# hhcho/sfgwas

Measured on AMD Instinct MI355X. Metric: pca_power_iter_ring_macs_per_s, higher is better.
Workload: dtype u64 ring words, exact integers: int8 digits on the matrix core for the MAC of all five moduli, fp64-held integers in the encode and key-switch kernels

## Files before the change

### sfgwas_amd/csrc/kernels.hpp

```cpp
#pragma once
#include "common.hpp"
#include "mm_plan.hpp"
#include "assoc_plan.hpp"

constexpr int SFG_MAXPATTERN = 128;
struct ModPattern { int period; int8_t m[SFG_MAXPATTERN]; };
struct RowMap { int rpg; size_t gstride_in, gstride_out; };
struct PanelMap { int G, g, shift0; unsigned packed_mask = 0; int K = 0; };

int launch_ntt_fwd(sfg_ctx *ctx, const u64 *in, u64 *out, size_t nrows, const ModPattern &pat);
int launch_ntt_inv(sfg_ctx *ctx, const u64 *in, u64 *out, size_t nrows, const ModPattern &pat);
int launch_ntt_plain(sfg_ctx *ctx, const double *pc, u64 *out, size_t nplain, int L);
struct MoveJob;
struct PtRide;
int launch_ntt_plain_half(sfg_ctx *ctx, const double *pc, u64 *out_half, size_t nplain, int L, PanelMap pm, const uint32_t *perm = nullptr, const MoveJob *mv = nullptr);
int launch_expand_half(sfg_ctx *ctx, const u64 *half, u64 *full, size_t nrows);
int launch_ntt_fwd_map(sfg_ctx *ctx, const u64 *in, u64 *out, size_t nrows, const ModPattern &pat, const RowMap &rm);
int launch_ntt_inv_map(sfg_ctx *ctx, const u64 *in, u64 *out, size_t nrows, const ModPattern &pat, const RowMap &rm);
int launch_ntt_fwd_staged(sfg_ctx *ctx, const u64 *in, u64 *out, size_t nrows, const ModPattern &pat, bool staged);
struct MacStrides { size_t rot_k, rot_r, pt_k, pt_n, out_n, out_r; bool pt_half = false; bool pt_packed = false; bool pt_digits = false; bool i8 = false; bool i8_big = false; bool pt_digits_big = false;
                    const int8_t *B_small = nullptr, *B_big = nullptr;
                    int pt_layout = 0, pt_L = 0;
                    int B_mode = 0;
                    const int8_t *A_small = nullptr, *A_big = nullptr; };
int launch_mac_i8_small(sfg_ctx *ctx, const double *rotf, size_t rotf_k_stride, size_t rotf_r_stride, int plane0, const u64 *pt, u64 *out, int K, int R, int r0, int Ncols,
                        int l0, int nl, int accumulate, const MacStrides &st);
int launch_mac_i8_big(sfg_ctx *ctx, const double *rotf, size_t rotf_k_stride, size_t rotf_r_stride, int plane0, const u64 *pt, u64 *out, int K, int R, int r0, int Ncols,
                      int l0, int accumulate, const MacStrides &st);
int launch_skew(sfg_ctx *ctx, const int8_t *blk, size_t ld, int r, int c, int transposed, int square, int8_t *D);
struct PcCache { double *slot = nullptr; int mode = 0; const uint32_t *perm = nullptr; };
int launch_encode_rows(sfg_ctx *ctx, const int8_t *D, int shift0, int nshift, int L, u64 *pt, bool half_rows = false, int G = 0, int g = 0, unsigned packed_mask = 0, const PcCache *pcache = nullptr,
                       PtRide *ride = nullptr);
int encode_rows_launches(const sfg_ctx *ctx, int nshift);
int i8_ride_prepare(sfg_ctx *ctx, const u64 *panel, int K, int Ncols, size_t pt_k, size_t pt_n, int layout, int L, int launches, PtRide &ride);
int i8_ride_finish(sfg_ctx *ctx, PtRide &ride);
int i8_ride_tiles(sfg_ctx *ctx, int K, int L, int8_t **Bs, int8_t **Bb);
struct I8Args;
void launch_i8_pack_pt_digits(hipStream_t q, const I8Args &a, unsigned items, bool big);
void launch_move_alone(hipStream_t q, const MoveJob &j);
int launch_share(sfg_ctx *ctx, const u64 *rows, size_t rows_ct_stride, const u64 *xr, size_t x_ct_stride, u64 *h, int nl, int nct);
int launch_add_rows(sfg_ctx *ctx, const u64 *a, size_t a_ct_stride, const u64 *b, size_t b_ct_stride, u64 *out, size_t out_ct_stride, int nl, int nct);
// ... 50 lines not shown
```

### sfgwas_amd/csrc/ntt.hip

```cpp
#include "common.hpp"
#include "kernels.hpp"
#include "i8_move.hpp"
#include "ntt_core.hpp"

template <int IN_MODE>
__global__ void __launch_bounds__(512) k_ntt_fwd(const void *in_, u64 *out_, ModPattern pat, RowMap rm, const double *tw_all, const double2 *pack_all, const ModConst *modc) {
    extern __shared__ double lds[];
    const int N = SFG_N, tid = threadIdx.x;
    const size_t row = blockIdx.x;
    const int m = pat.m[row % pat.period];
    const size_t grp = row / rm.rpg, gi = row % rm.rpg;
    if (m == -2) return;
    if (m < 0) {
        const u64 *src = (const u64 *)in_ + grp * rm.gstride_in + gi * N; u64 *dst = out_ + grp * rm.gstride_out + gi * N;
        if (IN_MODE == 0 && src != dst) for (int a = 0; a < 32; a++) dst[a * 512 + tid] = src[a * 512 + tid];
        return;
    }
    const double *tw = tw_all + (size_t)m * N;
    const double2 *pack = pack_all + (size_t)m * (N / 2);
    const double q = modc[m].q, qinv = modc[m].qinv;
    double v[32];
    if (IN_MODE == 0) {
        const u64 *in = (const u64 *)in_ + grp * rm.gstride_in + gi * N;
#pragma unroll
        for (int a = 0; a < 32; a++) v[a] = u64_to_f64(in[a * 512 + tid]);
    } else {
        const double *pc = (const double *)in_ + (row / pat.period) * (size_t)(N / 2);
#pragma unroll
        for (int a = 0; a < 16; a++) v[a] = pred(pc[a * 512 + tid], q, qinv);
#pragma unroll
        for (int a = 16; a < 32; a++) {
            int x = (a - 16) * 512 + tid;
            v[a] = x == 0 ? 0.0 : -pred(pc[N / 2 - x], q, qinv);
        }
    }
    ntt_fwd_phases(v, lds, tw, pack, q, qinv, tid);
    u64 *out = out_ + grp * rm.gstride_out + gi * N;
    {
        const int b = tid >> 4, c = tid & 15;
#pragma unroll
        for (int a = 0; a < 32; a++) out[a * 512 + tid] = f64_to_u64(canon(lds[a * LDS_ROW + c * 33 + b], q, qinv));
    }
}

__global__ void __launch_bounds__(512) k_ntt_inv(const u64 *in_, u64 *out_, ModPattern pat, RowMap rm, const double *tw_all, const double2 *pack_all, const ModConst *modc) {
    extern __shared__ double lds[];
    const int N = SFG_N, tid = threadIdx.x;
    const size_t row = blockIdx.x;
    const int m = pat.m[row % pat.period];
    if (m < 0) return;
    const size_t grp = row / rm.rpg, gi = row % rm.rpg;
    const double *tw = tw_all + (size_t)m * N;
    const double2 *pack = pack_all + (size_t)m * (N / 2);
    const double q = modc[m].q, qinv = modc[m].qinv;
    const u64 *in = in_ + grp * rm.gstride_in + gi * N;
    double v[32];
    {
        const int b = tid >> 4, c = tid & 15;
#pragma unroll
        for (int a = 0; a < 32; a++) lds[a * LDS_ROW + c * 33 + b] = u64_to_f64(in[a * 512 + tid]);
    }
    __syncthreads();
#pragma unroll
    for (int h = 0; h < 2; h++) {
        const int p = tid + 512 * h, a = p >> 5, b = p & 31;
        double w[16];
#pragma unroll
        for (int c = 0; c < 16; c++) w[c] = lds[a * LDS_ROW + c * 33 + b];
// ... 21 lines not shown
    {
        const int a = tid >> 4, c = tid & 15;
#pragma unroll
        for (int b = 0; b < 32; b++) v[b] = lds[a * LDS_ROW + c * 33 + b];
        gs_stage<32, 1>(v, q, qinv, [&](int g) { return tw[512 + a * 16 + g]; });
        gs_stage<32, 2>(v, q, qinv, [&](int g) { return tw[256 + a * 8 + g]; });
        gs_stage<32, 4>(v, q, qinv, [&](int g) { return tw[128 + a * 4 + g]; });
        gs_stage<32, 8>(v, q, qinv, [&](int g) { return tw[64 + a * 2 + g]; });
        gs_stage<32, 16>(v, q, qinv, [&](int g) { return tw[32 + a + g]; });
        __syncthreads();
#pragma unroll
        for (int b = 0; b < 32; b++) lds[a * LDS_ROW + b * 16 + c] = pred(v[b], q, qinv);
    }
    __syncthreads();
#pragma unroll
    for (int a = 0; a < 32; a++) v[a] = lds[a * LDS_ROW + tid];
    gs_stage<32, 1>(v, q, qinv, [&](int g) { return tw[16 + g]; });
    gs_stage<32, 2>(v, q, qinv, [&](int g) { return tw[8 + g]; });
    gs_stage<32, 4>(v, q, qinv, [&](int g) { return tw[4 + g]; });
    gs_stage<32, 8>(v, q, qinv, [&](int g) { return tw[2 + g]; });
    gs_stage<32, 16>(v, q, qinv, [&](int g) { return tw[1 + g]; });
    const double ninv = modc[m].ninv, ninv_q = modc[m].ninv_q;
    u64 *out = out_ + grp * rm.gstride_out + gi * N;
#pragma unroll
    for (int a = 0; a < 32; a++) {
        double x = mulmod_lazy(pred(v[a], q, qinv), ninv, ninv_q, q);
        out[a * 512 + tid] = f64_to_u64(canon(x, q, qinv));
    }
}

constexpr int H3_ROWA = 264;
constexpr int H3_WREG = 4 * 272;
constexpr int H3_DOUBLES = 16 * H3_ROWA > 4 * H3_WREG ? 16 * H3_ROWA : 4 * H3_WREG;
constexpr int H3_LDS_BYTES = H3_DOUBLES * 8;
struct NoFill {};
template <class First, class Store, class Fill = NoFill, bool WIDE = false>
__device__ __forceinline__ void ntt_half3_body(int hs, First first, Store store, double *lds, const double *tw, const double2 *pack, double q, double qinv, int tid, Fill fill = Fill()) {
    double v[32];
    const int a_b = tid >> 4, c_b = tid & 15;
    double w2[2][16];
    if constexpr (std::is_same<Fill, NoFill>::value) {
#pragma unroll
        for (int h = 0; h < 2; h++)
#pragma unroll
            for (int a = 0; a < 16; a++) w2[h][a] = first(a * 512 + tid + 256 * h);
    } else fill(w2);
// ... 201 lines not shown
    u64 *out = out_ + grp * rm.gstride_out + gi * N + (size_t)hs * n;
    if (m == -2) return;
    if (m < 0) {
        for (int k = 0; k < 32; k++) out[k * 256 + tid] = in[(size_t)hs * n + k * 256 + tid];
        return;
    }
    const double *tw = tw_all + (size_t)m * N;
    const double2 *pack = pack_all + (size_t)m * (N / 2);
    const double q = modc[m].q, qinv = modc[m].qinv;
    const double W = hs ? -tw[1] : tw[1], Wq = W * qinv;
    auto first = [&](int j) { return STAGED ? u64_to_f64(in[(size_t)hs * n + j]) : u64_to_f64(in[j]) + mulmod_lazy(u64_to_f64(in[n + j]), W, Wq, q); };
    ntt_half3_body(hs, first, [&](int j, double x) { out[j] = f64_to_u64(canon(x, q, qinv)); }, lds, tw, pack, q, qinv, tid);
}
__global__ void __launch_bounds__(256) k_expand_half(const u64 *half, u64 *full) {
    const int N = SFG_N, n = N / 2; const size_t row = blockIdx.x / (n / 256);
    const int i = (int)(blockIdx.x % (n / 256)) * 256 + threadIdx.x;
    const u64 v = half[row * n + i];
    full[row * N + i] = v; full[row * N + (N - 1 - i)] = v;
}

int ntt_set_attrs(sfg_ctx *ctx) {
    hipError_t e = hipFuncSetAttribute((const void *)k_ntt_fwd<0>, hipFuncAttributeMaxDynamicSharedMemorySize, LDS_DOUBLES * 8);
    if (e == hipSuccess) e = hipFuncSetAttribute((const void *)k_ntt_fwd<1>, hipFuncAttributeMaxDynamicSharedMemorySize, LDS_DOUBLES * 8);
    if (e == hipSuccess) e = hipFuncSetAttribute((const void *)k_ntt_inv, hipFuncAttributeMaxDynamicSharedMemorySize, LDS_DOUBLES * 8);
    if (e == hipSuccess) e = hipFuncSetAttribute((const void *)k_ntt_half3<false, false>, hipFuncAttributeMaxDynamicSharedMemorySize, H3_LDS_BYTES);
    if (e == hipSuccess) e = hipFuncSetAttribute((const void *)k_ntt_half3<true, false>, hipFuncAttributeMaxDynamicSharedMemorySize, H3_LDS_BYTES);
    if (e == hipSuccess) e = hipFuncSetAttribute((const void *)k_ntt_half3<false, true>, hipFuncAttributeMaxDynamicSharedMemorySize, H3_LDS_BYTES);
    if (e == hipSuccess) e = hipFuncSetAttribute((const void *)k_ntt_half3<true, true>, hipFuncAttributeMaxDynamicSharedMemorySize, H3_LDS_BYTES);
    if (e == hipSuccess) e = hipFuncSetAttribute((const void *)k_ntt_fwd_split<false>, hipFuncAttributeMaxDynamicSharedMemorySize, H3_LDS_BYTES);
    if (e == hipSuccess) e = hipFuncSetAttribute((const void *)k_ntt_fwd_split<true>, hipFuncAttributeMaxDynamicSharedMemorySize, H3_LDS_BYTES);
#define SFG_MV_ATTR(P, D, T) if (e == hipSuccess) e = hipFuncSetAttribute((const void *)k_ntt_half3_move<P, D, T>, hipFuncAttributeMaxDynamicSharedMemorySize, H3_LDS_BYTES)
    SFG_MV_ATTR(false, 1, true); SFG_MV_ATTR(true, 1, true);
#ifdef SFG_AB
    SFG_MV_ATTR(false, 1, false); SFG_MV_ATTR(false, 2, false); SFG_MV_ATTR(false, 2, true); SFG_MV_ATTR(false, 3, false); SFG_MV_ATTR(false, 3, true);
    SFG_MV_ATTR(true, 1, false); SFG_MV_ATTR(true, 2, false); SFG_MV_ATTR(true, 2, true); SFG_MV_ATTR(true, 3, false); SFG_MV_ATTR(true, 3, true);
    if (e == hipSuccess && ab_set_attrs(ctx)) return 1;
#endif
#undef SFG_MV_ATTR
    if (e != hipSuccess) SFG_FAIL(ctx, "cannot raise dynamic LDS limit for the NTT kernels");
    return 0;
}

static RowMap dense_map() { RowMap rm; rm.rpg = 1; rm.gstride_in = SFG_N; rm.gstride_out = SFG_N; return rm; }
int launch_ntt_fwd(sfg_ctx *ctx, const u64 *in, u64 *out, size_t nrows, const ModPattern &pat) { return launch_ntt_fwd_map(ctx, in, out, nrows, pat, dense_map()); }
int launch_ntt_inv(sfg_ctx *ctx, const u64 *in, u64 *out, size_t nrows, const ModPattern &pat) { return launch_ntt_inv_map(ctx, in, out, nrows, pat, dense_map()); }
int launch_ntt_fwd_map(sfg_ctx *ctx, const u64 *in, u64 *out, size_t nrows, const ModPattern &pat, const RowMap &rm) {
    if (!nrows) return 0;
// ... 41 lines not shown
        if (perm) SFG_TRY(launch_half3_move<true>(ctx, g2, pc, out_half, nplain, L, pm, perm, *mv));
        else SFG_TRY(launch_half3_move<false>(ctx, g2, pc, out_half, nplain, L, pm, (const uint32_t *)nullptr, *mv));
        SFG_HIP(ctx, hipGetLastError());
        return 0;
    }
    if (perm && dig) hipLaunchKernelGGL((k_ntt_half3<true, true>), grid, dim3(256), H3_LDS_BYTES, ctx->stream, pc, out_half, nplain, L, pm, ctx->tw_fwd, ctx->pack_fwd, ctx->modc, perm);
    else if (perm) hipLaunchKernelGGL((k_ntt_half3<true, false>), grid, dim3(256), H3_LDS_BYTES, ctx->stream, pc, out_half, nplain, L, pm, ctx->tw_fwd, ctx->pack_fwd, ctx->modc, perm);
    else if (dig) hipLaunchKernelGGL((k_ntt_half3<false, true>), grid, dim3(256), H3_LDS_BYTES, ctx->stream, pc, out_half, nplain, L, pm, ctx->tw_fwd, ctx->pack_fwd, ctx->modc, (const uint32_t *)nullptr);
#ifdef SFG_AB
    else if (ctx->cfg.ntt_half_full) ab_launch_ntt_half_full(ctx, pc, out_half, nplain, L, pm);
#endif
    else hipLaunchKernelGGL((k_ntt_half3<false, false>), grid, dim3(256), H3_LDS_BYTES, ctx->stream, pc, out_half, nplain, L, pm, ctx->tw_fwd, ctx->pack_fwd, ctx->modc, (const uint32_t *)nullptr);
    SFG_HIP(ctx, hipGetLastError());
    return 0;
}
int launch_expand_half(sfg_ctx *ctx, const u64 *half, u64 *full, size_t nrows) {
    if (!nrows) return 0;
    hipLaunchKernelGGL(k_expand_half, dim3((unsigned)(nrows * (SFG_N / 2 / 256))), dim3(256), 0, ctx->stream, half, full);
    SFG_HIP(ctx, hipGetLastError());
    return 0;
}
int launch_ntt_inv_map(sfg_ctx *ctx, const u64 *in, u64 *out, size_t nrows, const ModPattern &pat, const RowMap &rm) {
    if (!nrows) return 0;
    hipLaunchKernelGGL(k_ntt_inv, dim3((unsigned)nrows), dim3(512), LDS_DOUBLES * 8, ctx->stream, in, out, pat, rm, ctx->tw_inv, ctx->pack_inv, ctx->modc);
    SFG_HIP(ctx, hipGetLastError());
    return 0;
}

static int pattern_from_host(sfg_ctx *ctx, const int *mod_idx, int nrows, ModPattern &pat) {
    for (int period = 1; period <= 64 && period <= nrows; period++) {
        bool ok = true;
        for (int r = 0; r < nrows && ok; r++) ok = mod_idx[r] == mod_idx[r % period];
        if (ok) { pat.period = period; for (int i = 0; i < period; i++) { if (mod_idx[i] < 0 || mod_idx[i] >= ctx->nmod) SFG_FAIL(ctx, "modulus index out of range"); pat.m[i] = (int8_t)mod_idx[i]; } return 0; }
    }
    SFG_FAIL(ctx, "mod_idx must be periodic with period <= 64");
}

extern "C" int sfg_ntt_rows(sfg_ctx *ctx, uint64_t *rows, int nrows, const int *mod_idx) {
    SFG_HIP(ctx, hipSetDevice(ctx->device));
    ModPattern pat; SFG_TRY(pattern_from_host(ctx, mod_idx, nrows, pat));
    return launch_ntt_fwd(ctx, (const u64 *)rows, (u64 *)rows, nrows, pat);
}
extern "C" int sfg_intt_rows(sfg_ctx *ctx, uint64_t *rows, int nrows, const int *mod_idx) {
    SFG_HIP(ctx, hipSetDevice(ctx->device));
    ModPattern pat; SFG_TRY(pattern_from_host(ctx, mod_idx, nrows, pat));
    return launch_ntt_inv(ctx, (const u64 *)rows, (u64 *)rows, nrows, pat);
}
// ... 1 lines not shown
```

### sfgwas_amd/csrc/rotate.hip

```cpp
#include "common.hpp"
#include "kernels.hpp"
#include "ksw.hpp"


static void fill_ext(const sfg_ctx *ctx, ExtConst &e, const std::vector<int> &src) {
    memset(&e, 0, sizeof e);
    e.a = (int)src.size();
    for (int m = 0; m < e.a; m++) e.src[m] = src[m];
    for (int m = 0; m < e.a; m++) {
        u64 qm = ctx->q[src[m]], h = 1;
        for (int k = 0; k < e.a; k++) if (k != m) h = h_mulmod(h, ctx->q[src[k]] % qm, qm);
        u64 hi = h_invmod(h, qm);
        e.qhat_inv[m] = (double)hi; e.qhat_inv_q[m] = (double)hi / (double)qm;
    }
    for (int t = 0; t < ctx->nmod; t++) {
        u64 qt = ctx->q[t], D = 1 % qt;
        for (int m = 0; m < e.a; m++) {
            u64 ht = 1 % qt;
            for (int k = 0; k < e.a; k++) if (k != m) ht = h_mulmod(ht, ctx->q[src[k]] % qt, qt);
            e.qhat_t[t][m] = (double)ht; e.qhat_t_q[t][m] = (double)ht / (double)qt;
            D = h_mulmod(D, ctx->q[src[m]] % qt, qt);
        }
        e.D_t[t] = (double)D; e.D_t_q[t] = (double)D / (double)qt;
    }
}
// ... 111 lines not shown
    } else o[x] = (ff.centre && v > __builtin_floor(q * 0.5)) ? v - q : v;
}
__global__ void __launch_bounds__(256) k_ksw_finish(const u64 *ct_in, const int *inidx, const u64 *acc, const u64 *ext2, const uint16_t *const *index,
                                                   u64 *const *ct_out, const KswConst *kcp, const ModConst *modc, const u64 *add1, F64Form ff) {
    const KswConst &kc = *kcp;
    const int N = SFG_N, x = blockIdx.x * 256 + threadIdx.x, t = blockIdx.y; const size_t b = blockIdx.z;
    if (ff.on && t >= ff.L) return;
    const double q = modc[t].q, qinv = modc[t].qinv, pinv = kc.pinv[t], pinv_q = kc.pinv_q[t];
    const int src = index[b][x];
#pragma unroll
    for (int p = 0; p < 2; p++) {
        const double a = u64_to_f64(acc[((b * 2 + p) * (size_t)kc.nt + t) * N + src]);
        const double e = u64_to_f64(ext2[((b * 2 + p) * (size_t)kc.nl + t) * N + src]);
        double r = mulmod_lazy(a - e, pinv, pinv_q, q);
        if (p == 0) r += u64_to_f64(ct_in[((size_t)inidx[b] * 2 * (size_t)kc.nl + t) * N + src]);
        else if (add1) r += u64_to_f64(add1[((size_t)inidx[b] * (size_t)kc.nl + t) * N + src]);
        const double v = canon(r, q, qinv);
        if (ff.on) store_rot_f64(reinterpret_cast<double *>(ct_out[b]) + (size_t)p * ff.rowf, ff, t, x, v, q);
        else ct_out[b][((size_t)p * kc.nl + t) * N + x] = f64_to_u64(v);
    }
}

struct KswSeg { const u64 *plain; u64 *out; int start, count, accumulate, pad; };
__global__ void __launch_bounds__(256) k_ksw_finish_sum(const u64 *ct_in, const int *inidx, const u64 *acc, const u64 *ext2, const uint16_t *const *index,
                                                       const KswSeg *segs, const int *jobs, const KswConst *kcp, const ModConst *modc) {
    const KswConst &kc = *kcp;
    const int N = SFG_N, x = blockIdx.x * 256 + threadIdx.x, t = blockIdx.y;
    const KswSeg sg = segs[blockIdx.z];
    const double q = modc[t].q, qinv = modc[t].qinv, pinv = kc.pinv[t], pinv_q = kc.pinv_q[t];
    const size_t w0 = (size_t)t * N + x, w1 = ((size_t)kc.nl + t) * N + x;
    double s0 = 0.0, s1 = 0.0;
    if (sg.accumulate) { s0 = u64_to_f64(sg.out[w0]); s1 = u64_to_f64(sg.out[w1]); }
    if (sg.plain) { s0 += u64_to_f64(sg.plain[w0]); s1 += u64_to_f64(sg.plain[w1]); }
    for (int k = 0; k < sg.count; k++) {
        const size_t b = (size_t)jobs[sg.start + k];
        const int src = index[b][x];
        const double a0 = u64_to_f64(acc[((b * 2 + 0) * (size_t)kc.nt + t) * N + src]), e0 = u64_to_f64(ext2[((b * 2 + 0) * (size_t)kc.nl + t) * N + src]);
        const double a1 = u64_to_f64(acc[((b * 2 + 1) * (size_t)kc.nt + t) * N + src]), e1 = u64_to_f64(ext2[((b * 2 + 1) * (size_t)kc.nl + t) * N + src]);
        const double c0 = u64_to_f64(ct_in[((size_t)inidx[b] * 2 * (size_t)kc.nl + t) * N + src]);
        s0 += canon(mulmod_lazy(a0 - e0, pinv, pinv_q, q) + c0, q, qinv);
        s1 += canon(mulmod_lazy(a1 - e1, pinv, pinv_q, q), q, qinv);
        if ((k & 7) == 7) { s0 = pred(s0, q, qinv); s1 = pred(s1, q, qinv); }
    }
    sg.out[w0] = f64_to_u64(canon(s0, q, qinv)); sg.out[w1] = f64_to_u64(canon(s1, q, qinv));
}

__global__ void __launch_bounds__(256) k_ct_add(const u64 *a, const u64 *b, u64 *out, int nl, const ModConst *modc, size_t total_rows) {
    const int N = SFG_N; const size_t row = blockIdx.x / (N / 256); const int m = (int)(row % nl);
    const u64 q = modc[m].qi;
    const size_t off = row * N + (blockIdx.x % (N / 256)) * 256 + threadIdx.x;
    u64 v = a[off] + b[off]; out[off] = v >= q ? v - q : v;
}

struct KswSum { int nout; std::vector<int> group; std::vector<const u64 *> plain; u64 *out; size_t out_stride; int accumulate; };
static int launch_keyswitch_jobs(sfg_ctx *ctx, const u64 *in, int nin, int level, const std::vector<int> &job_in, const std::vector<const u64 *> &keyp,
                                 const std::vector<const uint16_t *> &idxp, const std::vector<u64 *> &outp, const u64 *add1, const F64Form *ffp = nullptr,
                                 const KswSum *sum = nullptr) {
    const int N = SFG_N, nl = level + 1;
    F64Form ff; memset(&ff, 0, sizeof ff); if (ffp) ff = *ffp;
    KswConst *kcd; KswConst kc;
    SFG_TRY(get_ksw(ctx, level, &kcd, &kc));
    const size_t ctw = (size_t)2 * nl * N;
    const int nr = (int)job_in.size(), nout = sum ? sum->nout : 0;
    if (sum && (ff.on || add1 || (int)sum->group.size() != nr || (int)sum->plain.size() != nout)) SFG_FAIL(ctx, "key switch: internal: malformed sum groups");
    if (!nr && !nout) return 0;
    const int nq_out = ff.on ? ff.L : nl;
    const bool pre1 = !ctx->cfg.ntt_fwd_full;
    const size_t in_rows = (size_t)nl + (size_t)kc.beta * kc.nt, job_rows = 2 * (size_t)kc.nt + 2 * (size_t)nl;
    const size_t budget = ctx->cfg.ksw_budget;
    int in_grp = (int)(budget / (in_rows * N * 8)); if (in_grp < 1) in_grp = 1; if (in_grp > nin) in_grp = nin;
    int chunk = (int)(budget / (job_rows * N * 8)); if (chunk < 1) chunk = 1; if (chunk > nr) chunk = nr;
    const size_t ptr_bytes = (size_t)nr * (3 * sizeof(void *) + 2 * sizeof(int)) + (size_t)nout * sizeof(KswSeg) + 256;
    const size_t ext_rows = (size_t)in_grp * kc.beta * kc.nt, ext2_rows = (size_t)chunk * 2 * nl;
    SFG_TRY(sfg_ws_reserve(ctx, (in_rows * in_grp + job_rows * chunk + ext_rows + ext2_rows) * N * 8 + ptr_bytes));
    u64 *c2 = (u64 *)ctx->ws, *ext = c2 + (size_t)in_grp * nl * N;
    u64 *acc = ext + ext_rows * N, *ext2 = acc + (size_t)chunk * 2 * kc.nt * N;
    u64 *extT = ext2 + ext2_rows * N, *ext2T = extT + ext_rows * N;
    const u64 **keys_all = (const u64 **)(ext2T + ext2_rows * N);
    const uint16_t **idx_all = (const uint16_t **)(keys_all + nr);
    u64 **out_all = (u64 **)(idx_all + nr);
    KswSeg *segs_d = (KswSeg *)(out_all + nr);
    int *inidx_all = (int *)(segs_d + nout);
    int *segjobs_d = inidx_all + nr;
    std::vector<char> seen(nout, 0);
    std::vector<KswSeg> segs; std::vector<int> segjobs;
    auto finish_sum = [&](const std::vector<int> &jobs, size_t c0, int nb, const u64 *bin, const int *inidx_d, const uint16_t **idx_d) -> int {
        std::vector<int> cnt(nout, 0), at(nout, 0);
        for (int k = 0; k < nb; k++) cnt[sum->group[jobs[c0 + k]]]++;
        segs.clear(); segjobs.assign(nb, 0);
        for (int i = 0, start = 0; i < nout; i++) {
            if (nb ? !cnt[i] : seen[i]) continue;
            KswSeg sg; sg.plain = seen[i] ? nullptr : sum->plain[i]; sg.out = sum->out + (size_t)i * sum->out_stride;
            sg.start = start; sg.count = cnt[i]; sg.accumulate = (sum->accumulate || seen[i]) ? 1 : 0; sg.pad = 0;
            at[i] = start; start += cnt[i]; seen[i] = 1; segs.push_back(sg);
        }
        for (int k = 0; k < nb; k++) segjobs[at[sum->group[jobs[c0 + k]]]++] = k;
        if (segs.empty()) return 0;
        SFG_TRY(sfg_upload_small(ctx, segs_d, segs.data(), segs.size() * sizeof(KswSeg)));
        SFG_TRY(sfg_upload_small(ctx, segjobs_d, segjobs.data(), (size_t)nb * sizeof(int)));
        hipLaunchKernelGGL(k_ksw_finish_sum, dim3(N / 256, nl, (unsigned)segs.size()), dim3(256), 0, ctx->stream, bin, inidx_d, acc, ext2T, idx_d, segs_d, segjobs_d, kcd, ctx->modc);
        SFG_HIP(ctx, hipGetLastError());
        return 0;
    };
    ModPattern pq; pq.period = nl; for (int m = 0; m < nl; m++) pq.m[m] = m < nq_out ? (int8_t)m : (int8_t)-2;
    ModPattern pin; pin.period = nl; for (int m = 0; m < nl; m++) pin.m[m] = (int8_t)m;
    ModPattern pext; pext.period = kc.beta * kc.nt;
    for (int i = 0; i < kc.beta; i++) for (int t = 0; t < kc.nt; t++)
        pext.m[i * kc.nt + t] = (kc.digit_of[t] == i || (t >= nq_out && t < nl)) ? (int8_t)-2 : (int8_t)kc.tmod[t];
    ModPattern pp; pp.period = kc.np; for (int p = 0; p < kc.np; p++) pp.m[p] = (int8_t)(ctx->nq + p);
    for (int i0 = 0; i0 < nin; i0 += in_grp) {
        const int ni = nin - i0 < in_grp ? nin - i0 : in_grp;
        std::vector<int> jobs;
        for (int k = 0; k < nr; k++) if (job_in[k] >= i0 && job_in[k] < i0 + ni) jobs.push_back(k);
        if (jobs.empty()) continue;
        const u64 *bin = in + (size_t)i0 * ctw;
        RowMap rm1; rm1.rpg = nl; rm1.gstride_in = ctw; rm1.gstride_out = (size_t)nl * N;
        SFG_TRY(launch_ntt_inv_map(ctx, bin + (size_t)nl * N, c2, (size_t)ni * nl, pin, rm1));
        if (pre1) hipLaunchKernelGGL(k_ksw_extend<true>, dim3(N / 512, kc.beta, ni), dim3(256), 0, ctx->stream, c2, ext, kcd, ctx->modc, ctx->tw_fwd);
        else hipLaunchKernelGGL(k_ksw_extend<false>, dim3(N / 512, kc.beta, ni), dim3(256), 0, ctx->stream, c2, ext, kcd, ctx->modc, ctx->tw_fwd);
        SFG_HIP(ctx, hipGetLastError());
        SFG_TRY(launch_ntt_fwd_staged(ctx, ext, extT, (size_t)ni * kc.beta * kc.nt, pext, pre1));
        {
            const size_t nj = jobs.size();
            std::vector<const u64 *> kp(nj); std::vector<const uint16_t *> ip(nj); std::vector<u64 *> op(nj); std::vector<int> ii(nj);
            for (size_t k = 0; k < nj; k++) { int jb = jobs[k]; kp[k] = keyp[jb]; ip[k] = idxp[jb]; op[k] = sum ? nullptr : outp[jb]; ii[k] = job_in[jb] - i0; }
            SFG_TRY(sfg_upload_small(ctx, keys_all, kp.data(), nj * sizeof(void *)));
            SFG_TRY(sfg_upload_small(ctx, idx_all, ip.data(), nj * sizeof(void *)));
            if (!sum) SFG_TRY(sfg_upload_small(ctx, out_all, op.data(), nj * sizeof(void *)));
            SFG_TRY(sfg_upload_small(ctx, inidx_all, ii.data(), nj * sizeof(int)));
        }
        for (size_t c0 = 0; c0 < jobs.size(); c0 += chunk) {
            const int nb = (int)(jobs.size() - c0 < (size_t)chunk ? jobs.size() - c0 : (size_t)chunk);
            const u64 **keys_d = keys_all + c0; const uint16_t **idx_d = idx_all + c0; u64 **out_d = out_all + c0; int *inidx_d = inidx_all + c0;
            hipLaunchKernelGGL(k_ksw_inner, dim3(N / 512, nq_out + kc.np, nb), dim3(256), 0, ctx->stream, extT, bin, keys_d, inidx_d, acc, kcd, ctx->modc, ctx->nmod, nq_out);
            SFG_HIP(ctx, hipGetLastError());
            RowMap rm4; rm4.rpg = kc.np; rm4.gstride_in = (size_t)kc.nt * N; rm4.gstride_out = (size_t)kc.nt * N;
            SFG_TRY(launch_ntt_inv_map(ctx, acc + (size_t)nl * N, acc + (size_t)nl * N, (size_t)nb * 2 * kc.np, pp, rm4));
            if (pre1) hipLaunchKernelGGL(k_moddown_extend<true>, dim3(N / 512, 2, nb), dim3(256), 0, ctx->stream, acc, ext2, kcd, ctx->modc, ctx->tw_fwd, nq_out);
            else hipLaunchKernelGGL(k_moddown_extend<false>, dim3(N / 512, 2, nb), dim3(256), 0, ctx->stream, acc, ext2, kcd, ctx->modc, ctx->tw_fwd, nq_out);
            SFG_HIP(ctx, hipGetLastError());
            SFG_TRY(launch_ntt_fwd_staged(ctx, ext2, ext2T, (size_t)nb * 2 * nl, pq, pre1));
            if (sum) { SFG_TRY(finish_sum(jobs, c0, nb, bin, inidx_d, idx_d)); continue; }
            hipLaunchKernelGGL(k_ksw_finish, dim3(N / 256, nq_out, nb), dim3(256), 0, ctx->stream, bin, inidx_d, acc, ext2T, idx_d, out_d, kcd, ctx->modc,
                               add1 ? add1 + (size_t)i0 * nl * N : nullptr, ff);
            SFG_HIP(ctx, hipGetLastError());
        }
    }
    if (sum) SFG_TRY(finish_sum(std::vector<int>(), 0, 0, in, inidx_all, idx_all));
    return 0;
}
int launch_rotate_right_indexed(sfg_ctx *ctx, const u64 *in, int nin, u64 *out, int nct, int level, const int *nrot_host, const int *in_index) {
    const int N = SFG_N, nl = level + 1;
    if (level < 0 || level >= ctx->nq) SFG_FAIL(ctx, "rotate: level out of range");
    const size_t ctw = (size_t)2 * nl * N;
    std::vector<int> job_in; std::vector<const u64 *> keyp; std::vector<const uint16_t *> idxp; std::vector<u64 *> outp;
    for (int j = 0; j < nct; j++) {
        int nrot = nrot_host[j] % SFG_SLOTS; if (nrot < 0) nrot += SFG_SLOTS;
        const int src = in_index ? in_index[j] : j;
        if (src < 0 || src >= nin) SFG_FAIL(ctx, "rotate: input index out of range");
        if (nrot == 0) {
            int run = 1;
            while (j + run < nct && (nrot_host[j + run] % SFG_SLOTS) == 0 && (in_index ? in_index[j + run] : j + run) == src + run && src + run < nin) run++;
            SFG_HIP(ctx, hipMemcpyAsync(out + j * ctw, in + (size_t)src * ctw, (size_t)run * ctw * 8, hipMemcpyDeviceToDevice, ctx->stream));
            j += run - 1;
            continue;
        }
        u64 g = sfg_galois_for_rotation(ctx, SFG_SLOTS - nrot);
        auto it = ctx->rotkeys().find(g);
        if (it == ctx->rotkeys().end()) SFG_FAIL(ctx, "rotate: no rotation key loaded for right-rotation by %d (galois element %llu)", nrot, g);
        job_in.push_back(src); keyp.push_back(it->second.key_dev); idxp.push_back(it->second.index_dev); outp.push_back(out + j * ctw);
    }
    return launch_keyswitch_jobs(ctx, in, nin, level, job_in, keyp, idxp, outp, nullptr);
}
int launch_rotate_right_sum(sfg_ctx *ctx, const u64 *in, int nin, int nct, int level, const int *nrot_host, const int *in_index, const int *group, int nout,
                            u64 *out, size_t out_stride, int accumulate) {
    const int N = SFG_N, nl = level + 1;
    if (level < 0 || level >= ctx->nq) SFG_FAIL(ctx, "rotate: level out of range");
    const size_t ctw = (size_t)2 * nl * N;
    KswSum sum; sum.nout = nout; sum.plain.assign(nout, nullptr); sum.out = out; sum.out_stride = out_stride; sum.accumulate = accumulate;
    std::vector<int> job_in; std::vector<const u64 *> keyp; std::vector<const uint16_t *> idxp;
    for (int j = 0; j < nct; j++) {
        int nrot = nrot_host[j] % SFG_SLOTS; if (nrot < 0) nrot += SFG_SLOTS;
        const int src = in_index ? in_index[j] : j;
        if (src < 0 || src >= nin) SFG_FAIL(ctx, "rotate: input index out of range");
        if (group[j] < 0 || group[j] >= nout) SFG_FAIL(ctx, "rotate: sum group out of range");
        if (nrot == 0) {
            if (sum.plain[group[j]]) SFG_FAIL(ctx, "rotate: more than one unrotated member in a sum group");
            sum.plain[group[j]] = in + (size_t)src * ctw;
            continue;
        }
        u64 g = sfg_galois_for_rotation(ctx, SFG_SLOTS - nrot);
        auto it = ctx->rotkeys().find(g);
        if (it == ctx->rotkeys().end()) SFG_FAIL(ctx, "rotate: no rotation key loaded for right-rotation by %d (galois element %llu)", nrot, g);
        job_in.push_back(src); keyp.push_back(it->second.key_dev); idxp.push_back(it->second.index_dev); sum.group.push_back(group[j]);
    }
    return launch_keyswitch_jobs(ctx, in, nin, level, job_in, keyp, idxp, std::vector<u64 *>(), nullptr, nullptr, &sum);
}
int launch_rotate_right_indexed_f64(sfg_ctx *ctx, const u64 *in, int nin, double *outf, int nct, int level, const int *nrot_host, const int *in_index, int L,
                                    const size_t *out_slot) {
    const int N = SFG_N, nl = level + 1;
    ctx->i8_gen++;
    if (level < 0 || level >= ctx->nq || L > nl) SFG_FAIL(ctx, "rotate: level out of range");
    const size_t ctw = (size_t)2 * nl * N;
    std::vector<int> plane_of, is_big; const int nplanes = mac_dma_planes(ctx, L, plane_of, is_big);
    if (nplanes < 0) return 1;
    F64Form ff; memset(&ff, 0, sizeof ff);
    ff.on = 1; ff.L = L; ff.centre = mac_dma_packed_mask(ctx, L) != 0; ff.rowf = (size_t)nplanes * N;
    for (int l = 0; l < L; l++) { ff.plane_of[l] = plane_of[l]; ff.big[l] = is_big[l]; }
    std::vector<int> job_in; std::vector<const u64 *> keyp; std::vector<const uint16_t *> idxp; std::vector<u64 *> outp;
    for (int j = 0; j < nct; j++) {
        int nrot = nrot_host[j] % SFG_SLOTS; if (nrot < 0) nrot += SFG_SLOTS;
        const int src = in_index ? in_index[j] : j;
        if (src < 0 || src >= nin) SFG_FAIL(ctx, "rotate: input index out of range");
        double *dst = outf + (out_slot ? out_slot[j] : (size_t)j) * 2 * ff.rowf;
        if (nrot == 0) {
            int run = 1;
            while (!out_slot && j + run < nct && (nrot_host[j + run] % SFG_SLOTS) == 0 && (in_index ? in_index[j + run] : j + run) == src + run && src + run < nin) run++;
// ... 61 lines not shown
```

Baseline: 6113 billion.

## Sum rotated key-switch outputs before mod-down by applying the Galois map in coefficient domain

For rotate-and-sum groups, the inverse NTT of the P-part now writes each coefficient at its Galois-permuted position and tags negated ones. A new kernel then does mod-down extension and summation across the group's jobs, split over a few partial sums, before a single forward NTT per partial. The finish kernel sums raw accumulators and divides by P once. This removes a forward NTT and an extension per job in exchange for a scatter through LDS, extra partial-sum buffers and more workspace.

Result: no change. 6156 billion (median of 6 runs) (+0.7%).

```diff
diff --git a/sfgwas_amd/csrc/galois_coeff.hpp b/sfgwas_amd/csrc/galois_coeff.hpp
--- /dev/null
+++ b/sfgwas_amd/csrc/galois_coeff.hpp
@@ -0,0 +1,12 @@
+#pragma once
+#include "fp64mod.hpp"
+
+SFG_HD void galois_coeff_dst(unsigned i, unsigned g, unsigned n, unsigned &j, unsigned &neg) {
+    const unsigned r = (i * g) & (2u * n - 1u);
+    j = r & (n - 1u); neg = r >= n ? 1u : 0u;
+}
+constexpr unsigned long long GALOIS_NEG = 1ull << 63;
+SFG_HD unsigned long long galois_tag(unsigned long long word, unsigned neg) { return neg ? word | GALOIS_NEG : word; }
+SFG_HD unsigned galois_neg_of(unsigned long long tagged) { return (unsigned)(tagged >> 63); }
+SFG_HD unsigned long long galois_word_of(unsigned long long tagged) { return tagged & ~GALOIS_NEG; }
+SFG_HD double galois_signed(double v, unsigned neg, double q) { return neg ? (v != 0.0 ? q - v : 0.0) : v; }
diff --git a/sfgwas_amd/csrc/kernels.hpp b/sfgwas_amd/csrc/kernels.hpp
--- a/sfgwas_amd/csrc/kernels.hpp
+++ b/sfgwas_amd/csrc/kernels.hpp
@@ -17,6 +17,7 @@
 int launch_expand_half(sfg_ctx *ctx, const u64 *half, u64 *full, size_t nrows);
 int launch_ntt_fwd_map(sfg_ctx *ctx, const u64 *in, u64 *out, size_t nrows, const ModPattern &pat, const RowMap &rm);
 int launch_ntt_inv_map(sfg_ctx *ctx, const u64 *in, u64 *out, size_t nrows, const ModPattern &pat, const RowMap &rm);
+int launch_ntt_inv_galois(sfg_ctx *ctx, const u64 *in, u64 *out, size_t nrows, const ModPattern &pat, const RowMap &rm, const unsigned *galois_dev, int gal_rows);
 int launch_ntt_fwd_staged(sfg_ctx *ctx, const u64 *in, u64 *out, size_t nrows, const ModPattern &pat, bool staged);
 struct MacStrides { size_t rot_k, rot_r, pt_k, pt_n, out_n, out_r; bool pt_half = false; bool pt_packed = false; bool pt_digits = false; bool i8 = false; bool i8_big = false; bool pt_digits_big = false;
                     const int8_t *B_small = nullptr, *B_big = nullptr;
diff --git a/sfgwas_amd/csrc/ntt.hip b/sfgwas_amd/csrc/ntt.hip
--- a/sfgwas_amd/csrc/ntt.hip
+++ b/sfgwas_amd/csrc/ntt.hip
@@ -2,6 +2,7 @@
 #include "kernels.hpp"
 #include "i8_move.hpp"
 #include "ntt_core.hpp"
+#include "galois_coeff.hpp"
 
 template <int IN_MODE>
 __global__ void __launch_bounds__(512) k_ntt_fwd(const void *in_, u64 *out_, ModPattern pat, RowMap rm, const double *tw_all, const double2 *pack_all, const ModConst *modc) {
@@ -43,7 +44,9 @@
     }
 }
 
-__global__ void __launch_bounds__(512) k_ntt_inv(const u64 *in_, u64 *out_, ModPattern pat, RowMap rm, const double *tw_all, const double2 *pack_all, const ModConst *modc) {
+template <bool GAL>
+__global__ void __launch_bounds__(512) k_ntt_inv(const u64 *in_, u64 *out_, ModPattern pat, RowMap rm, const double *tw_all, const double2 *pack_all, const ModConst *modc,
+                                                 const unsigned *galois, int gal_rows) {
     extern __shared__ double lds[];
     const int N = SFG_N, tid = threadIdx.x;
     const size_t row = blockIdx.x;
@@ -111,6 +114,21 @@
     gs_stage<32, 16>(v, q, qinv, [&](int g) { return tw[1 + g]; });
     const double ninv = modc[m].ninv, ninv_q = modc[m].ninv_q;
     u64 *out = out_ + grp * rm.gstride_out + gi * N;
+    if (GAL) {
+        const unsigned g = galois[row / (size_t)gal_rows];
+        u64 *img = reinterpret_cast<u64 *>(lds);
+        __syncthreads();
+#pragma unroll
+        for (int a = 0; a < 32; a++) {
+            double x = mulmod_lazy(pred(v[a], q, qinv), ninv, ninv_q, q);
+            unsigned j, neg; galois_coeff_dst((unsigned)(a * 512 + tid), g, (unsigned)N, j, neg);
+            img[(j >> 9) * LDS_ROW + (j & 511)] = galois_tag(f64_to_u64(canon(x, q, qinv)), neg);
+        }
+        __syncthreads();
+#pragma unroll
+        for (int a = 0; a < 32; a++) out[a * 512 + tid] = img[a * LDS_ROW + tid];
+        return;
+    }
 #pragma unroll
     for (int a = 0; a < 32; a++) {
         double x = mulmod_lazy(pred(v[a], q, qinv), ninv, ninv_q, q);
@@ -358,7 +376,8 @@
 int ntt_set_attrs(sfg_ctx *ctx) {
     hipError_t e = hipFuncSetAttribute((const void *)k_ntt_fwd<0>, hipFuncAttributeMaxDynamicSharedMemorySize, LDS_DOUBLES * 8);
     if (e == hipSuccess) e = hipFuncSetAttribute((const void *)k_ntt_fwd<1>, hipFuncAttributeMaxDynamicSharedMemorySize, LDS_DOUBLES * 8);
-    if (e == hipSuccess) e = hipFuncSetAttribute((const void *)k_ntt_inv, hipFuncAttributeMaxDynamicSharedMemorySize, LDS_DOUBLES * 8);
+    if (e == hipSuccess) e = hipFuncSetAttribute((const void *)k_ntt_inv<false>, hipFuncAttributeMaxDynamicSharedMemorySize, LDS_DOUBLES * 8);
+    if (e == hipSuccess) e = hipFuncSetAttribute((const void *)k_ntt_inv<true>, hipFuncAttributeMaxDynamicSharedMemorySize, LDS_DOUBLES * 8);
     if (e == hipSuccess) e = hipFuncSetAttribute((const void *)k_ntt_half3<false, false>, hipFuncAttributeMaxDynamicSharedMemorySize, H3_LDS_BYTES);
     if (e == hipSuccess) e = hipFuncSetAttribute((const void *)k_ntt_half3<true, false>, hipFuncAttributeMaxDynamicSharedMemorySize, H3_LDS_BYTES);
     if (e == hipSuccess) e = hipFuncSetAttribute((const void *)k_ntt_half3<false, true>, hipFuncAttributeMaxDynamicSharedMemorySize, H3_LDS_BYTES);
@@ -446,7 +465,14 @@
 }
 int launch_ntt_inv_map(sfg_ctx *ctx, const u64 *in, u64 *out, size_t nrows, const ModPattern &pat, const RowMap &rm) {
     if (!nrows) return 0;
-    hipLaunchKernelGGL(k_ntt_inv, dim3((unsigned)nrows), dim3(512), LDS_DOUBLES * 8, ctx->stream, in, out, pat, rm, ctx->tw_inv, ctx->pack_inv, ctx->modc);
+    hipLaunchKernelGGL(k_ntt_inv<false>, dim3((unsigned)nrows), dim3(512), LDS_DOUBLES * 8, ctx->stream, in, out, pat, rm, ctx->tw_inv, ctx->pack_inv, ctx->modc, (const unsigned *)nullptr, 1);
+    SFG_HIP(ctx, hipGetLastError());
+    return 0;
+}
+int launch_ntt_inv_galois(sfg_ctx *ctx, const u64 *in, u64 *out, size_t nrows, const ModPattern &pat, const RowMap &rm, const unsigned *galois_dev, int gal_rows) {
+    if (!nrows) return 0;
+    if (!galois_dev || gal_rows < 1) SFG_FAIL(ctx, "inverse NTT: the automorphism store needs a Galois element per job");
+    hipLaunchKernelGGL(k_ntt_inv<true>, dim3((unsigned)nrows), dim3(512), LDS_DOUBLES * 8, ctx->stream, in, out, pat, rm, ctx->tw_inv, ctx->pack_inv, ctx->modc, galois_dev, gal_rows);
     SFG_HIP(ctx, hipGetLastError());
     return 0;
 }
diff --git a/sfgwas_amd/csrc/rotate.hip b/sfgwas_amd/csrc/rotate.hip
--- a/sfgwas_amd/csrc/rotate.hip
+++ b/sfgwas_amd/csrc/rotate.hip
@@ -1,6 +1,7 @@
 #include "common.hpp"
 #include "kernels.hpp"
 #include "ksw.hpp"
+#include "galois_coeff.hpp"
 
 
 static void fill_ext(const sfg_ctx *ctx, ExtConst &e, const std::vector<int> &src) {
@@ -158,25 +159,81 @@
 }
 
 struct KswSeg { const u64 *plain; u64 *out; int start, count, accumulate, pad; };
-__global__ void __launch_bounds__(256) k_ksw_finish_sum(const u64 *ct_in, const int *inidx, const u64 *acc, const u64 *ext2, const uint16_t *const *index,
-                                                       const KswSeg *segs, const int *jobs, const KswConst *kcp, const ModConst *modc) {
+constexpr int KSW_SUM_PARTS = 8;
+constexpr int KSW_SUM_WGS = 4096;
+template <bool PRE1, int MAXT>
+__global__ void __launch_bounds__(256) k_moddown_extend_sum(const u64 *acc, u64 *esum, const KswSeg *segs, const int *jobs, const KswConst *kcp, const ModConst *modc,
+                                                           const double *tw_fwd, int nq_out, int nparts) {
+    const KswConst &kc = *kcp;
+    const int N = SFG_N, n = N / 2, x = blockIdx.x * 256 + threadIdx.x, p = blockIdx.y;
+    const KswSeg sg = segs[blockIdx.z / nparts];
+    const ExtConst &e = kc.pq;
+    double s[2][MAXT];
+#pragma unroll
+    for (int t = 0; t < MAXT; t++) s[0][t] = s[1][t] = 0.0;
+    for (int k = blockIdx.z % nparts, c = 0; k < sg.count; k += nparts, c++) {
+        const size_t b = (size_t)jobs[sg.start + k];
+        const u64 *ap = acc + ((b * 2 + p) * (size_t)kc.nt + kc.nl) * N;
+        double xs[2][KSW_MAXA], y[2][KSW_MAXA], v[2] = {0.0, 0.0};
+        unsigned neg[2] = {0u, 0u};
+#pragma unroll
+        for (int h = 0; h < 2; h++)
+#pragma unroll
+            for (int m = 0; m < KSW_MAXA; m++) {
+                const u64 w = m < e.a ? ap[(size_t)m * N + h * n + x] : 0;
+                xs[h][m] = u64_to_f64(galois_word_of(w));
+                if (m == 0) neg[h] = galois_neg_of(w);
+            }
+        if (e.a > 1) { ext_prepare(e, modc, xs[0], y[0], v[0]); ext_prepare(e, modc, xs[1], y[1], v[1]); }
+#pragma unroll
+        for (int t = 0; t < MAXT; t++) {
+            if (t < nq_out) {
+                const double q = modc[t].q, qinv = modc[t].qinv;
+                double o0, o1;
+                if (e.a == 1) { o0 = canon(xs[0][0], q, qinv); o1 = canon(xs[1][0], q, qinv); }
+                else { o0 = ext_target(e, t, q, qinv, y[0], v[0]); o1 = ext_target(e, t, q, qinv, y[1], v[1]); }
+                s[0][t] += galois_signed(o0, neg[0], q); s[1][t] += galois_signed(o1, neg[1], q);
+                if ((c & 7) == 7) { s[0][t] = pred(s[0][t], q, qinv); s[1][t] = pred(s[1][t], q, qinv); }
+            }
+        }
+    }
+#pragma unroll
+    for (int t = 0; t < MAXT; t++) {
+        if (t < nq_out) {
+            const double q = modc[t].q, qinv = modc[t].qinv;
+            double o0 = canon(s[0][t], q, qinv), o1 = canon(s[1][t], q, qinv);
+            if (PRE1) { const double W = tw_fwd[(size_t)t * N + 1]; fwd_stage1_pair(o0, o1, W, W * qinv, q, qinv, o0, o1); }
+            u64 *row = esum + (((size_t)blockIdx.z * 2 + p) * (size_t)kc.nl + t) * N;
+            row[x] = f64_to_u64(o0); row[n + x] = f64_to_u64(o1);
+        }
+    }
+}
+__global__ void __launch_bounds__(256) k_ksw_finish_sum(const u64 *ct_in, const int *inidx, const u64 *acc, const u64 *esumT, const uint16_t *const *index,
+                                                       const KswSeg *segs, const int *jobs, const KswConst *kcp, const ModConst *modc, int nparts) {
     const KswConst &kc = *kcp;
     const int N = SFG_N, x = blockIdx.x * 256 + threadIdx.x, t = blockIdx.y;
     const KswSeg sg = segs[blockIdx.z];
     const double q = modc[t].q, qinv = modc[t].qinv, pinv = kc.pinv[t], pinv_q = kc.pinv_q[t];
     const size_t w0 = (size_t)t * N + x, w1 = ((size_t)kc.nl + t) * N + x;
-    double s0 = 0.0, s1 = 0.0;
+    double s0 = 0.0, s1 = 0.0, a0 = 0.0, a1 = 0.0;
     if (sg.accumulate) { s0 = u64_to_f64(sg.out[w0]); s1 = u64_to_f64(sg.out[w1]); }
     if (sg.plain) { s0 += u64_to_f64(sg.plain[w0]); s1 += u64_to_f64(sg.plain[w1]); }
     for (int k = 0; k < sg.count; k++) {
         const size_t b = (size_t)jobs[sg.start + k];
         const int src = index[b][x];
-        const double a0 = u64_to_f64(acc[((b * 2 + 0) * (size_t)kc.nt + t) * N + src]), e0 = u64_to_f64(ext2[((b * 2 + 0) * (size_t)kc.nl + t) * N + src]);
-        const double a1 = u64_to_f64(acc[((b * 2 + 1) * (size_t)kc.nt + t) * N + src]), e1 = u64_to_f64(ext2[((b * 2 + 1) * (size_t)kc.nl + t) * N + src]);
-        const double c0 = u64_to_f64(ct_in[((size_t)inidx[b] * 2 * (size_t)kc.nl + t) * N + src]);
-        s0 += canon(mulmod_lazy(a0 - e0, pinv, pinv_q, q) + c0, q, qinv);
-        s1 += canon(mulmod_lazy(a1 - e1, pinv, pinv_q, q), q, qinv);
-        if ((k & 7) == 7) { s0 = pred(s0, q, qinv); s1 = pred(s1, q, qinv); }
+        a0 += u64_to_f64(acc[((b * 2 + 0) * (size_t)kc.nt + t) * N + src]);
+        a1 += u64_to_f64(acc[((b * 2 + 1) * (size_t)kc.nt + t) * N + src]);
+        s0 += u64_to_f64(ct_in[((size_t)inidx[b] * 2 * (size_t)kc.nl + t) * N + src]);
+        if ((k & 7) == 7) { a0 = pred(a0, q, qinv); a1 = pred(a1, q, qinv); s0 = pred(s0, q, qinv); }
+    }
+    if (sg.count) {
+        double e0 = 0.0, e1 = 0.0;
+        for (int r = 0; r < nparts; r++) {
+            e0 += u64_to_f64(esumT[((((size_t)blockIdx.z * nparts + r) * 2 + 0) * (size_t)kc.nl + t) * N + x]);
+            e1 += u64_to_f64(esumT[((((size_t)blockIdx.z * nparts + r) * 2 + 1) * (size_t)kc.nl + t) * N + x]);
+        }
+        s0 += mulmod_lazy(pred(a0, q, qinv) - e0, pinv, pinv_q, q);
+        s1 += mulmod_lazy(pred(a1, q, qinv) - e1, pinv, pinv_q, q);
     }
     sg.out[w0] = f64_to_u64(canon(s0, q, qinv)); sg.out[w1] = f64_to_u64(canon(s1, q, qinv));
 }
@@ -188,7 +245,7 @@
     u64 v = a[off] + b[off]; out[off] = v >= q ? v - q : v;
 }
 
-struct KswSum { int nout; std::vector<int> group; std::vector<const u64 *> plain; u64 *out; size_t out_stride; int accumulate; };
+struct KswSum { int nout; std::vector<int> group; std::vector<unsigned> galois; std::vector<const u64 *> plain; u64 *out; size_t out_stride; int accumulate; };
 static int launch_keyswitch_jobs(sfg_ctx *ctx, const u64 *in, int nin, int level, const std::vector<int> &job_in, const std::vector<const u64 *> &keyp,
                                  const std::vector<const uint16_t *> &idxp, const std::vector<u64 *> &outp, const u64 *add1, const F64Form *ffp = nullptr,
                                  const KswSum *sum = nullptr) {
@@ -198,7 +255,7 @@
     SFG_TRY(get_ksw(ctx, level, &kcd, &kc));
     const size_t ctw = (size_t)2 * nl * N;
     const int nr = (int)job_in.size(), nout = sum ? sum->nout : 0;
-    if (sum && (ff.on || add1 || (int)sum->group.size() != nr || (int)sum->plain.size() != nout)) SFG_FAIL(ctx, "key switch: internal: malformed sum groups");
+    if (sum && (ff.on || add1 || (int)sum->group.size() != nr || (int)sum->galois.size() != nr || (int)sum->plain.size() != nout)) SFG_FAIL(ctx, "key switch: internal: malformed sum groups");
     if (!nr && !nout) return 0;
     const int nq_out = ff.on ? ff.L : nl;
     const bool pre1 = !ctx->cfg.ntt_fwd_full;
@@ -206,9 +263,10 @@
     const size_t budget = ctx->cfg.ksw_budget;
     int in_grp = (int)(budget / (in_rows * N * 8)); if (in_grp < 1) in_grp = 1; if (in_grp > nin) in_grp = nin;
     int chunk = (int)(budget / (job_rows * N * 8)); if (chunk < 1) chunk = 1; if (chunk > nr) chunk = nr;
-    const size_t ptr_bytes = (size_t)nr * (3 * sizeof(void *) + 2 * sizeof(int)) + (size_t)nout * sizeof(KswSeg) + 256;
-    const size_t ext_rows = (size_t)in_grp * kc.beta * kc.nt, ext2_rows = (size_t)chunk * 2 * nl;
-    SFG_TRY(sfg_ws_reserve(ctx, (in_rows * in_grp + job_rows * chunk + ext_rows + ext2_rows) * N * 8 + ptr_bytes));
+    const size_t ptr_bytes = (size_t)nr * (3 * sizeof(void *) + 3 * sizeof(int)) + (size_t)nout * sizeof(KswSeg) + 256;
+    const int sum_sets = sum ? std::max(std::min(nout * KSW_SUM_PARTS, chunk), 1) : 0;
+    const size_t ext_rows = (size_t)in_grp * kc.beta * kc.nt, ext2_rows = (size_t)(sum ? sum_sets : chunk) * 2 * nl;
+    SFG_TRY(sfg_ws_reserve(ctx, (in_rows * in_grp + (size_t)chunk * 2 * kc.nt + ext_rows + 2 * ext2_rows) * N * 8 + ptr_bytes));
     u64 *c2 = (u64 *)ctx->ws, *ext = c2 + (size_t)in_grp * nl * N;
     u64 *acc = ext + ext_rows * N, *ext2 = acc + (size_t)chunk * 2 * kc.nt * N;
     u64 *extT = ext2 + ext2_rows * N, *ext2T = extT + ext_rows * N;
@@ -218,9 +276,13 @@
     KswSeg *segs_d = (KswSeg *)(out_all + nr);
     int *inidx_all = (int *)(segs_d + nout);
     int *segjobs_d = inidx_all + nr;
+    unsigned *gal_all = (unsigned *)(segjobs_d + nr);
     std::vector<char> seen(nout, 0);
     std::vector<KswSeg> segs; std::vector<int> segjobs;
-    auto finish_sum = [&](const std::vector<int> &jobs, size_t c0, int nb, const u64 *bin, const int *inidx_d, const uint16_t **idx_d) -> int {
+    ModPattern pq; pq.period = nl; for (int m = 0; m < nl; m++) pq.m[m] = m < nq_out ? (int8_t)m : (int8_t)-2;
+    ModPattern pp; pp.period = kc.np; for (int p = 0; p < kc.np; p++) pp.m[p] = (int8_t)(ctx->nq + p);
+    RowMap rm4; rm4.rpg = kc.np; rm4.gstride_in = (size_t)kc.nt * N; rm4.gstride_out = (size_t)kc.nt * N;
+    auto finish_sum = [&](const std::vector<int> &jobs, size_t c0, int nb, const u64 *bin, const int *inidx_d, const uint16_t **idx_d, const unsigned *gal_d) -> int {
         std::vector<int> cnt(nout, 0), at(nout, 0);
         for (int k = 0; k < nb; k++) cnt[sum->group[jobs[c0 + k]]]++;
         segs.clear(); segjobs.assign(nb, 0);
@@ -234,16 +296,26 @@
         if (segs.empty()) return 0;
         SFG_TRY(sfg_upload_small(ctx, segs_d, segs.data(), segs.size() * sizeof(KswSeg)));
         SFG_TRY(sfg_upload_small(ctx, segjobs_d, segjobs.data(), (size_t)nb * sizeof(int)));
-        hipLaunchKernelGGL(k_ksw_finish_sum, dim3(N / 256, nl, (unsigned)segs.size()), dim3(256), 0, ctx->stream, bin, inidx_d, acc, ext2T, idx_d, segs_d, segjobs_d, kcd, ctx->modc);
+        const int nseg = (int)segs.size(); int nparts = 1;
+        if (nb) {
+            SFG_TRY(launch_ntt_inv_galois(ctx, acc + (size_t)nl * N, acc + (size_t)nl * N, (size_t)nb * 2 * kc.np, pp, rm4, gal_d, 2 * kc.np));
+            nparts = std::max(1, std::min(std::min(KSW_SUM_PARTS, (KSW_SUM_WGS + 63) / (64 * nseg)), sum_sets / nseg));
+            const dim3 grid(N / 512, 2, (unsigned)(nseg * nparts));
+#define SFG_EXT_SUM(P, T) hipLaunchKernelGGL((k_moddown_extend_sum<P, T>), grid, dim3(256), 0, ctx->stream, acc, ext2, segs_d, segjobs_d, kcd, ctx->modc, ctx->tw_fwd, nq_out, nparts)
+            if (nq_out <= 8) { if (pre1) SFG_EXT_SUM(true, 8); else SFG_EXT_SUM(false, 8); }
+            else { if (pre1) SFG_EXT_SUM(true, SFG_MAXMOD); else SFG_EXT_SUM(false, SFG_MAXMOD); }
+#undef SFG_EXT_SUM
+            SFG_HIP(ctx, hipGetLastError());
+            SFG_TRY(launch_ntt_fwd_staged(ctx, ext2, ext2T, (size_t)nseg * nparts * 2 * nl, pq, pre1));
+        }
+        hipLaunchKernelGGL(k_ksw_finish_sum, dim3(N / 256, nl, (unsigned)segs.size()), dim3(256), 0, ctx->stream, bin, inidx_d, acc, ext2T, idx_d, segs_d, segjobs_d, kcd, ctx->modc, nparts);
         SFG_HIP(ctx, hipGetLastError());
         return 0;
     };
-    ModPattern pq; pq.period = nl; for (int m = 0; m < nl; m++) pq.m[m] = m < nq_out ? (int8_t)m : (int8_t)-2;
     ModPattern pin; pin.period = nl; for (int m = 0; m < nl; m++) pin.m[m] = (int8_t)m;
     ModPattern pext; pext.period = kc.beta * kc.nt;
     for (int i = 0; i < kc.beta; i++) for (int t = 0; t < kc.nt; t++)
         pext.m[i * kc.nt + t] = (kc.digit_of[t] == i || (t >= nq_out && t < nl)) ? (int8_t)-2 : (int8_t)kc.tmod[t];
-    ModPattern pp; pp.period = kc.np; for (int p = 0; p < kc.np; p++) pp.m[p] = (int8_t)(ctx->nq + p);
     for (int i0 = 0; i0 < nin; i0 += in_grp) {
         const int ni = nin - i0 < in_grp ? nin - i0 : in_grp;
         std::vector<int> jobs;
@@ -264,25 +336,29 @@
             SFG_TRY(sfg_upload_small(ctx, idx_all, ip.data(), nj * sizeof(void *)));
             if (!sum) SFG_TRY(sfg_upload_small(ctx, out_all, op.data(), nj * sizeof(void *)));
             SFG_TRY(sfg_upload_small(ctx, inidx_all, ii.data(), nj * sizeof(int)));
+            if (sum) {
+                std::vector<unsigned> gl(nj);
+                for (size_t k = 0; k < nj; k++) gl[k] = sum->galois[jobs[k]];
+                SFG_TRY(sfg_upload_small(ctx, gal_all, gl.data(), nj * sizeof(unsigned)));
+            }
         }
         for (size_t c0 = 0; c0 < jobs.size(); c0 += chunk) {
             const int nb = (int)(jobs.size() - c0 < (size_t)chunk ? jobs.size() - c0 : (size_t)chunk);
             const u64 **keys_d = keys_all + c0; const uint16_t **idx_d = idx_all + c0; u64 **out_d = out_all + c0; int *inidx_d = inidx_all + c0;
             hipLaunchKernelGGL(k_ksw_inner, dim3(N / 512, nq_out + kc.np, nb), dim3(256), 0, ctx->stream, extT, bin, keys_d, inidx_d, acc, kcd, ctx->modc, ctx->nmod, nq_out);
             SFG_HIP(ctx, hipGetLastError());
-            RowMap rm4; rm4.rpg = kc.np; rm4.gstride_in = (size_t)kc.nt * N; rm4.gstride_out = (size_t)kc.nt * N;
+            if (sum) { SFG_TRY(finish_sum(jobs, c0, nb, bin, inidx_d, idx_d, gal_all + c0)); continue; }
             SFG_TRY(launch_ntt_inv_map(ctx, acc + (size_t)nl * N, acc + (size_t)nl * N, (size_t)nb * 2 * kc.np, pp, rm4));
             if (pre1) hipLaunchKernelGGL(k_moddown_extend<true>, dim3(N / 512, 2, nb), dim3(256), 0, ctx->stream, acc, ext2, kcd, ctx->modc, ctx->tw_fwd, nq_out);
             else hipLaunchKernelGGL(k_moddown_extend<false>, dim3(N / 512, 2, nb), dim3(256), 0, ctx->stream, acc, ext2, kcd, ctx->modc, ctx->tw_fwd, nq_out);
             SFG_HIP(ctx, hipGetLastError());
             SFG_TRY(launch_ntt_fwd_staged(ctx, ext2, ext2T, (size_t)nb * 2 * nl, pq, pre1));
-            if (sum) { SFG_TRY(finish_sum(jobs, c0, nb, bin, inidx_d, idx_d)); continue; }
             hipLaunchKernelGGL(k_ksw_finish, dim3(N / 256, nq_out, nb), dim3(256), 0, ctx->stream, bin, inidx_d, acc, ext2T, idx_d, out_d, kcd, ctx->modc,
                                add1 ? add1 + (size_t)i0 * nl * N : nullptr, ff);
             SFG_HIP(ctx, hipGetLastError());
         }
     }
-    if (sum) SFG_TRY(finish_sum(std::vector<int>(), 0, 0, in, inidx_all, idx_all));
+    if (sum) SFG_TRY(finish_sum(std::vector<int>(), 0, 0, in, inidx_all, idx_all, gal_all));
     return 0;
 }
 int launch_rotate_right_indexed(sfg_ctx *ctx, const u64 *in, int nin, u64 *out, int nct, int level, const int *nrot_host, const int *in_index) {
@@ -328,7 +404,7 @@
         u64 g = sfg_galois_for_rotation(ctx, SFG_SLOTS - nrot);
         auto it = ctx->rotkeys().find(g);
         if (it == ctx->rotkeys().end()) SFG_FAIL(ctx, "rotate: no rotation key loaded for right-rotation by %d (galois element %llu)", nrot, g);
-        job_in.push_back(src); keyp.push_back(it->second.key_dev); idxp.push_back(it->second.index_dev); sum.group.push_back(group[j]);
+        job_in.push_back(src); keyp.push_back(it->second.key_dev); idxp.push_back(it->second.index_dev); sum.group.push_back(group[j]); sum.galois.push_back((unsigned)g);
     }
     return launch_keyswitch_jobs(ctx, in, nin, level, job_in, keyp, idxp, std::vector<u64 *>(), nullptr, nullptr, &sum);
 }
```
